# jason-li-831202/Vehicle-CV-ADAS

Hardware: NVIDIA H100
Metric: end-to-end frames/sec (YOLOv8l+UFLDv2+ByteTrack) 1280x720 (higher is better)
Workload: dtype f16

## Files before the change

vehicle-cv-adas_b200/csrc/gemm_v3.cu:

```cuda
#include "common.h"
#include <math.h>
#include <stdlib.h>
#include <string.h>
#include <mutex>
#include "tc_common.cuh"
#include "gemm_v3.h"

namespace adas {

template <bool HS>
__device__ __forceinline__ float v3_act(float x, int act) {
    if constexpr (HS) return hardswish(x);
    else return act_apply_base(x, act);
}

template <int BN, bool UP2, bool HS>
__global__ void __launch_bounds__(V3_THREADS, 1)
conv_gemm_v3_kernel(const __grid_constant__ CUtensorMap tmA, const __grid_constant__ CUtensorMap tmB, const GemmV3 g) {
    constexpr int MTX = V3_ACC_COLS / BN >= 4 ? 4 : V3_ACC_COLS / BN >= 1 ? V3_ACC_COLS / BN : 1;
    extern __shared__ uint8_t smem_raw[];
    __shared__ __align__(8) uint64_t full_bar[8];
    __shared__ __align__(8) uint64_t empty_bar[8];

    const GemmParams& p = g.p;
    const int warp_idx = threadIdx.x >> 5;
    const int lane = threadIdx.x & 31;
    const int stages = g.stages;
    const uint32_t smem_base = (smem_u32(smem_raw) + 1023u) & ~1023u;
    const int BMT = BM * g.MT;

    if (threadIdx.x == 0) {
        asm volatile("prefetch.tensormap [%0];" ::"l"(reinterpret_cast<uint64_t>(&tmA)) : "memory");
        asm volatile("prefetch.tensormap [%0];" ::"l"(reinterpret_cast<uint64_t>(&tmB)) : "memory");
        for (int s = 0; s < stages; ++s) {
            mbar_init(smem_u32(&full_bar[s]), 1);
            mbar_init(smem_u32(&empty_bar[s]), 4 * V3_CONSUMERS);
        }
        asm volatile("fence.mbarrier_init.release.cluster;" ::: "memory");
        asm volatile("fence.proxy.async.shared::cta;" ::: "memory");
    }
    __syncthreads();
    const int tps = g.slab ? 3 : 1;
    const uint32_t a_bytes = p.s2 ? (uint32_t)(p.s2_bw * p.s2_bh * BK * 2) : (uint32_t)g.a_sub_bytes;
    const uint32_t tx_bytes = (uint32_t)g.MT * a_bytes + (uint32_t)(tps * BN * BK * 2);
    const bool dx_inner = p.ntaps == 9;
    const int o_cnt = dx_inner ? 3 : p.ntaps;
    const int i_cnt = dx_inner && !g.slab ? 3 : 1;
    const int per_img = p.s2_tw * p.s2_th;
    auto load_b = [&](int grp, int kc, int n0, uint32_t stage, uint32_t fb) {
        const uint32_t b_dst = smem_base + stage * g.stage_bytes + g.MT * g.a_sub_bytes;
        for (int t = 0; t < tps; ++t) tma_load_2d(b_dst + t * g.b_bytes, &tmB, (grp + t) * p.Kc + kc * BK, n0, fb);
    };
    auto load_a = [&](int grp, int kc, int m_t, uint32_t stage, uint32_t fb) {
        const uint32_t a_dst = smem_base + stage * g.stage_bytes;
        const int m0 = m_t * BMT;
        if (p.s2) {
            const int dy = p.ntaps == 9 ? grp / 3 : 1, dx = p.ntaps == 9 ? grp % 3 : 1;
            for (int mt = 0; mt < g.MT; ++mt) {
                const int pi = m_t * g.MT + mt;
                const int b = pi / per_img;
                const int rem = pi - b * per_img;
                const int ty = rem / p.s2_tw, tx = rem - ty * p.s2_tw;
                tma_load_4d(a_dst + mt * g.a_sub_bytes, &tmA, kc * BK, 2 * tx * p.s2_bw + dx, 2 * ty * p.s2_bh + dy, b, fb);
            }
        } else {
            int shift = 0;
            if (p.ntaps == 9) shift = (grp / 3 - 1) * p.Wp + (grp % 3 - 1);
            else if (p.ntaps == 4) shift = (grp - 2) * p.Wp;
            for (int mt = 0; mt < g.MT; ++mt) tma_load_2d(a_dst + mt * g.a_sub_bytes, &tmA, kc * BK, m0 + shift + mt * BM, fb);
        }
    };
    int pre = 0;
    if (threadIdx.x == 0 && g.pdl && g.prefetch_w && (int)blockIdx.x < g.total_tiles) {
        const int steps_tile = o_cnt * p.kpt * i_cnt;
        pre = steps_tile < stages ? steps_tile : stages;
        const int n0 = ((int)blockIdx.x % g.n_tiles) * BN;
        for (int j = 0; j < pre; ++j) {
            const int in = j % i_cnt, kc = (j / i_cnt) % p.kpt, o = j / (i_cnt * p.kpt);
            const uint32_t fb = smem_u32(&full_bar[j]);
            mbar_expect_tx(fb, tx_bytes);
            load_b(dx_inner ? o * 3 + in : o, kc, n0, (uint32_t)j, fb);
        }
    }
    if (g.pdl) {
        asm volatile("griddepcontrol.wait;" ::: "memory");
        asm volatile("griddepcontrol.launch_dependents;" ::: "memory");
    }

    if (warp_idx < 4) {
        asm volatile("setmaxnreg.dec.sync.aligned.u32 40;" ::: "memory");
        if (threadIdx.x == 0) {
            uint32_t s = 0, ph = 0;
            int step = 0;
            for (int w = blockIdx.x; w < g.total_tiles; w += gridDim.x) {
                const int n_t = w % g.n_tiles, m_t = w / g.n_tiles;
                const int n0 = n_t * BN;
                for (int o = 0; o < o_cnt; ++o) {
                    for (int kc = 0; kc < p.kpt; ++kc) {
                        for (int in = 0; in < i_cnt; ++in) {
                            const int grp = dx_inner ? o * 3 + in : o;
                            const uint32_t fb = smem_u32(&full_bar[s]);
                            if (step < pre) {
                                load_a(grp, kc, m_t, s, fb);
                            } else {
                                mbar_wait(smem_u32(&empty_bar[s]), ph ^ 1u);
                                mbar_expect_tx(fb, tx_bytes);
                                load_a(grp, kc, m_t, s, fb);
                                load_b(grp, kc, n0, s, fb);
                            }
                            ++step;
                            if (++s == (uint32_t)stages) { s = 0; ph ^= 1u; }
                        }
                    }
                }
            }
        }
    } else {
        asm volatile("setmaxnreg.inc.sync.aligned.u32 232;" ::: "memory");
        const int cw = (warp_idx - 4) >> 2;
        const int wq = warp_idx & 3;
        const int nsteps = p.ntaps * p.kpt / tps;
        const size_t res_ld = (size_t)(p.res_ld < 0 ? -p.res_ld : p.res_ld);
        float acc[MTX][BN / 2];
#pragma unroll
        for (int mt = 0; mt < MTX; ++mt)
#pragma unroll
            for (int i = 0; i < BN / 2; ++i) acc[mt][i] = 0.f;
        uint32_t s = 0, ph = 0;
        for (int w = blockIdx.x; w < g.total_tiles; w += gridDim.x) {
            uint32_t prev = 0;
            for (int ks = 0; ks < nsteps; ++ks) {
                mbar_wait(smem_u32(&full_bar[s]), ph);
                const uint32_t a_base = smem_base + s * g.stage_bytes + (uint32_t)cw * (64u * 128u);
                const uint32_t b_base = smem_base + s * g.stage_bytes + g.MT * g.a_sub_bytes;
#pragma unroll
                for (int mt = 0; mt < MTX; ++mt)
#pragma unroll
                    for (int i = 0; i < BN / 2; ++i) reg_fence(acc[mt][i]);
                wgmma_fence();
                for (int t = 0; t < tps; ++t) {
                    const uint64_t bdesc = make_smem_desc(b_base + t * g.b_bytes);
#pragma unroll
                    for (int mt = 0; mt < MTX; ++mt) {
                        if (mt < g.MT) {
                            const uint64_t adesc = make_smem_desc(a_base + (uint32_t)(mt * g.a_sub_bytes + t * 128));
#pragma unroll
                            for (int k = 0; k < BK / 16; ++k)
                                WgmmaCols<0, BN>::run(acc[mt], adesc + 2u * k, bdesc + 2u * k, (uint32_t)((ks | t | k) != 0));
                        }
                    }
                }
                wgmma_commit();
                wgmma_wait<1>();
                if (ks > 0 && lane == 0) mbar_arrive(smem_u32(&empty_bar[prev]));
                prev = s;
                if (++s == (uint32_t)stages) { s = 0; ph ^= 1u; }
            }
            wgmma_wait<0>();
#pragma unroll
            for (int mt = 0; mt < MTX; ++mt)
#pragma unroll
                for (int i = 0; i < BN / 2; ++i) reg_fence(acc[mt][i]);
            if (lane == 0) mbar_arrive(smem_u32(&empty_bar[prev]));

            const int n_t = w % g.n_tiles, m_t = w / g.n_tiles;
            const int n0 = n_t * BN;
            const int m0 = m_t * BMT;
            const int c0 = 2 * (lane & 3);
            const float neg_slope = p.act == 3 ? 0.1f : 0.f;
#pragma unroll
            for (int mt = 0; mt < MTX; ++mt) {
                if (mt >= g.MT) break;
#pragma unroll
                for (int h = 0; h < 2; ++h) {
                    const int r = cw * 64 + wq * 16 + (lane >> 2) + 8 * h;
                    int row = m0 + mt * BM + r;
                    bool ok = row < p.M;
                    if (p.s2) {
                        const int pi = m_t * g.MT + mt;
                        const int b = fast_div(pi, g.fd_per_img);
                        const int rem = pi - b * per_img;
                        const int ty = fast_div(rem, g.fd_tw), tx = rem - ty * p.s2_tw;
                        const int j = fast_div(r, g.fd_bw), i = r - j * p.s2_bw;
                        const int yo = ty * p.s2_bh + j, xo = tx * p.s2_bw + i;
                        ok = (pi < g.n_patches) && (r < p.s2_bw * p.s2_bh) && (yo < p.s2_Ho) && (xo < p.s2_Wo);
                        row = (b * (p.s2_Ho + 2) + yo + 1) * (p.s2_Wo + 2) + xo + 1;
                    } else if (p.mask_H > 0 && ok) {
                        const int Wp = p.mask_W + 2;
                        const int pp = row - fast_div(row, g.fd_img) * g.fd_img.d;
                        const int yy = fast_div(pp, g.fd_wp);
                        const int xx = pp - yy * Wp;
                        ok = (yy >= 1) && (yy <= p.mask_H) && (xx >= 1) && (xx <= p.mask_W);
                    }
                    if (!ok) continue;
                    if (p.transposed) {
                        const float row_bias = p.bias != nullptr ? __ldg(p.bias + row) : 0.f;
#pragma unroll
                        for (int j = 0; j < BN / 8; ++j) {
#pragma unroll
                            for (int e = 0; e < 2; ++e) {
                                const int col = n0 + 8 * j + c0 + e;
                                if (col < p.N) {
                                    const float x = v3_act<HS>(acc[mt][4 * j + 2 * h + e] + row_bias, p.act);
                                    if (p.out_f32) reinterpret_cast<float*>(p.out)[(size_t)col * (size_t)p.out_ld + row] = x;
                                    else reinterpret_cast<__half*>(p.out)[(size_t)col * (size_t)p.out_ld + row] = __float2half_rn(x);
                                }
                            }
                        }
                        continue;
                    }
                    if constexpr (UP2) {
                        const int bi = fast_div(row, g.fd_img);
                        const int pp = row - bi * g.fd_img.d;
                        const int yy = fast_div(pp, g.fd_wp), xx = pp - yy * (p.mask_W + 2);
                        const int Wo2 = 2 * p.mask_W + 2, co = p.N >> 2;
                        const int up_row = (bi * (2 * p.mask_H + 2) + 2 * yy - 1) * Wo2 + 2 * xx - 1;
#pragma unroll
                        for (int j = 0; j < BN / 8; ++j) {
                            const int n = n0 + 8 * j + c0;
                            if (n0 + 8 * j >= p.N) break;
                            float x0 = acc[mt][4 * j + 2 * h], x1 = acc[mt][4 * j + 2 * h + 1];
                            if (p.bias != nullptr) { x0 += __ldg(p.bias + n); x1 += __ldg(p.bias + n + 1); }
                            x0 = v3_act<HS>(x0, p.act); x1 = v3_act<HS>(x1, p.act);
                            const int q = (n >= co) + (n >= 2 * co) + (n >= 3 * co);
                            const size_t o = (size_t)(up_row + (q >> 1) * Wo2 + (q & 1)) * (size_t)p.out_ld + (n - q * co);
                            if (p.out_f32) *reinterpret_cast<float2*>(reinterpret_cast<float*>(p.out) + o) = make_float2(x0, x1);
                            else *reinterpret_cast<__half2*>(reinterpret_cast<__half*>(p.out) + o) = __floats2half2_rn(x0, x1);
                        }
                        continue;
                    }
                    const __half* rp = p.res != nullptr ? p.res + (size_t)row * res_ld : nullptr;
#pragma unroll
                    for (int j = 0; j < BN / 8; ++j) {
                        const int n = n0 + 8 * j + c0;
                        if (n0 + 8 * j >= p.N) break;
                        float x0 = acc[mt][4 * j + 2 * h], x1 = acc[mt][4 * j + 2 * h + 1];
                        if (p.bias != nullptr) { x0 += __ldg(p.bias + n); x1 += __ldg(p.bias + n + 1); }
                        float2 rv = make_float2(0.f, 0.f);
                        if (rp != nullptr) rv = __half22float2(*reinterpret_cast<const __half2*>(rp + n));
                        if (p.res_ld < 0) { x0 += rv.x; x1 += rv.y; }
                        if constexpr (HS) { x0 = hardswish(x0); x1 = hardswish(x1); }
                        else if (p.act == 1) silu2(x0, x1);
                        else if (p.act >= 2) { x0 = relu_leaky(x0, neg_slope); x1 = relu_leaky(x1, neg_slope); }
                        if (p.res_ld > 0) { x0 += p.res_scale * rv.x; x1 += p.res_scale * rv.y; }
                        if (p.out_f32) *reinterpret_cast<float2*>(reinterpret_cast<float*>(p.out) + (size_t)row * (size_t)p.out_ld + n) = make_float2(x0, x1);
                        else *reinterpret_cast<__half2*>(reinterpret_cast<__half*>(p.out) + (size_t)row * (size_t)p.out_ld + n) = __floats2half2_rn(x0, x1);
                    }
                }
            }
        }
    }
}

#define V3_FOR_EACH_BN(X) X(16) X(32) X(48) X(64) X(80) X(96) X(112) X(128) X(144) X(160) X(176) X(192) X(208) X(224) X(240) X(256)

template <bool HS>
static const void* v3_kernel_act(int BN, bool up2) {
    if (up2) {
        switch (BN) {
            case 64: return reinterpret_cast<const void*>(&conv_gemm_v3_kernel<64, true, HS>);
            case 128: return reinterpret_cast<const void*>(&conv_gemm_v3_kernel<128, true, HS>);
            case 256: return reinterpret_cast<const void*>(&conv_gemm_v3_kernel<256, true, HS>);
            default: return nullptr;
        }
    }
    switch (BN) {
#define V3_CASE(b) case b: return reinterpret_cast<const void*>(&conv_gemm_v3_kernel<b, false, HS>);
        V3_FOR_EACH_BN(V3_CASE)
#undef V3_CASE
        default: return nullptr;
    }
}
static const void* v3_kernel(int BN, bool up2 = false, bool hswish = false) {
    return hswish ? v3_kernel_act<true>(BN, up2) : v3_kernel_act<false>(BN, up2);
}
static bool v3_up2_tile(int BN) { return BN == 64 || BN == 128 || BN == 256; }

struct V3Device { bool attr_set = false; int num_sms = 0; };
static std::mutex g_v3_mu;
static V3Device g_v3_dev[64];

static int v3_device_state(int* num_sms) {
    int dev = 0;
    ADAS_CUDA(cudaGetDevice(&dev));
    ADAS_CHECK(dev >= 0 && dev < 64, "device index %d out of range", dev);
    std::lock_guard<std::mutex> lk(g_v3_mu);
    V3Device& d = g_v3_dev[dev];
    if (!d.attr_set) {
        for (int hs = 0; hs < 2; ++hs) {
            for (int bn = 16; bn <= 256; bn += 16) ADAS_CUDA(cudaFuncSetAttribute(v3_kernel(bn, false, hs), cudaFuncAttributeMaxDynamicSharedMemorySize, V3_DYN_SMEM_MAX));
            for (int bn = 64; bn <= 256; bn *= 2) ADAS_CUDA(cudaFuncSetAttribute(v3_kernel(bn, true, hs), cudaFuncAttributeMaxDynamicSharedMemorySize, V3_DYN_SMEM_MAX));
        }
        ADAS_CUDA(cudaDeviceGetAttribute(&d.num_sms, cudaDevAttrMultiProcessorCount, dev));
        d.attr_set = true;
    }
    *num_sms = d.num_sms;
    return 0;
}

static FastDiv make_fastdiv(int d) {
    FastDiv f;
    f.d = d < 1 ? 1 : d;
    f.mul = 0; f.shr = 0;
    if (f.d > 1) {
        int lg = 0;
        while ((1u << lg) < (uint32_t)f.d) ++lg;
        const int p = 31 + lg;
        f.mul = (uint32_t)((((uint64_t)1 << p) + (uint64_t)f.d - 1) / (uint64_t)f.d);
        f.shr = (uint32_t)(p - 32);
    }
    return f;
}

int v3_num_sms(int* num_sms) { return v3_device_state(num_sms); }

static int env_int(const char* name, int dflt) {
    const char* v = getenv(name);
    return v ? atoi(v) : dflt;
}

int gemm_v3_config(const GemmParams& p_in, GemmV3* g) {
    GemmParams p = p_in;
    static const int force_bn = env_int("ADAS_B200_BN", 0), force_mt = env_int("ADAS_B200_MT", 0);
    if (force_bn >= 16 && force_bn <= 256 && force_bn % 16 == 0 && force_bn <= ((p.N + 15) / 16) * 16 && !p.transposed && !p.up2) p.BN = force_bn;
    if (p.BN % 16 != 0 || p.BN < 16 || p.BN > 256) return 1;
    if (p.up2 && !v3_up2_tile(p.BN)) return 1;
    g->p = p;
    g->MT = p.mt_hint >= 1 ? p.mt_hint : ((p.BN <= 128) ? 2 : 1);
    if (force_mt >= 1 && force_mt <= 4) g->MT = force_mt;
    if (g->MT > 4) return 1;
    const int mt_max = V3_ACC_COLS / p.BN < 4 ? V3_ACC_COLS / p.BN : 4;
    if (g->MT > mt_max) g->MT = mt_max;
    const int b_bytes = ((p.BN * BK * 2) + 1023) & ~1023;
    g->b_bytes = b_bytes;
    static const int no_slab_env = env_int("ADAS_B200_NOSLAB", 0);
    const int slab_stage = g->MT * SLAB_BYTES + 3 * b_bytes;
    g->slab = p.ntaps == 9 && !p.s2 && !p.no_slab && !no_slab_env && 2 * slab_stage <= V3_DYN_SMEM_MAX - 1024;
    g->a_sub_bytes = g->slab ? SLAB_BYTES : A_STAGE_BYTES;
    g->stage_bytes = g->slab ? slab_stage : g->MT * g->a_sub_bytes + b_bytes;
    int stages = (V3_DYN_SMEM_MAX - 1024) / g->stage_bytes;
    if (stages > 8) stages = 8;
    if (stages < 2) return 1;
    g->stages = stages;
    g->p.stages = stages;
    const int BMT = BM * g->MT;
    g->n_tiles = (p.N + p.BN - 1) / p.BN;
    g->m_tiles = (p.M + BMT - 1) / BMT;
    g->total_tiles = g->n_tiles * g->m_tiles;
    g->n_patches = p.s2 ? p.M / BM : 0;
    g->fd_img = make_fastdiv((p.mask_H + 2) * (p.mask_W + 2));
    g->fd_wp = make_fastdiv(p.mask_W + 2);
    g->fd_per_img = make_fastdiv(p.s2 ? p.s2_tw * p.s2_th : 1);
    g->fd_tw = make_fastdiv(p.s2 ? p.s2_tw : 1);
    g->fd_bw = make_fastdiv(p.s2 ? p.s2_bw : 1);
    g->pdl = 0;
    static const int no_prefetch = env_int("ADAS_B200_NO_WPREFETCH", 0);
    g->prefetch_w = (no_prefetch || p.transposed) ? 0 : 1;
    return 0;
}

static int v3_smem_bytes(const GemmV3& g) { return g.stages * g.stage_bytes + 1024; }

int gemm_v3_launch(const GemmV3Launch& L, cudaStream_t st) {
    int num_sms = 0;
    if (v3_device_state(&num_sms)) return 1;
    static const int pdl = env_int("ADAS_B200_PDL", 1);
    GemmV3 gp = L.g;
    gp.pdl = pdl ? 1 : 0;
    const void* fn = v3_kernel(gp.p.BN, gp.p.up2 != 0, gp.p.act == 5);
    ADAS_CHECK(fn != nullptr, "gemm_v3: no kernel for BN %d%s", gp.p.BN, gp.p.up2 ? " with the transposed-conv store" : "");
    cudaLaunchConfig_t cfg = {};
    cfg.gridDim = dim3(gp.total_tiles < num_sms ? gp.total_tiles : num_sms, 1, 1);
    cfg.blockDim = dim3(V3_THREADS, 1, 1);
    cfg.dynamicSmemBytes = v3_smem_bytes(gp);
    cfg.stream = st;
    cudaLaunchAttribute attr1;
    attr1.id = cudaLaunchAttributeProgrammaticStreamSerialization;
    attr1.val.programmaticStreamSerializationAllowed = 1;
    cfg.attrs = &attr1;
    cfg.numAttrs = pdl ? 1 : 0;
    CUtensorMap tmA = L.tmA, tmB = L.tmB;
    void* args[] = {&tmA, &tmB, &gp};
    ADAS_CUDA(cudaLaunchKernelExC(&cfg, fn, args));
    count_launch();
    return 0;
}

int gemm_v3_candidates(const GemmParams& base, int max_out, int* BN_out, int* mt_out, int* no_slab_out) {
    int num_sms = 132;
    if (v3_num_sms(&num_sms)) return 0;
    const int cand[] = {256, 192, 128, 64, 160, 96, 80, 48, 32, 16};
    struct C { double t; int BN, mt, slab; } list[64];
    int n = 0;
    const int N = base.N, ntaps = base.ntaps;
    const int kpt = (base.Kc + 63) / 64;
    for (int ci = 0; ci < 10; ++ci) {
        int BN = cand[ci];
        if (BN > N) { if (BN - N >= 64 || (BN % 64 == 0 && BN - N >= 16 && N > 64)) continue; BN = (N + 15) / 16 * 16; }
        if (BN > 256) continue;
        if (BN < 64 && N >= 64) continue;
        if (base.up2 && !v3_up2_tile(BN)) continue;
        const int n_tiles = (N + BN - 1) / BN;
        if ((double)n_tiles * BN > 1.35 * N) continue;
        bool dup = false;
        for (int k = 0; k < n; ++k) dup = dup || (list[k].BN == BN);
        if (dup) continue;
        for (int mt = 1; mt <= 4; ++mt) {
            GemmParams p = base;
            p.BN = BN; p.mt_hint = mt;
            GemmV3 g;
            if (gemm_v3_config(p, &g)) continue;
            if (g.p.BN != BN || g.MT != mt) continue;
            const double tiles = (double)g.total_tiles;
            const int tps = g.slab ? 3 : 1;
            const double bytes = (double)ntaps * kpt / tps * (g.MT * (double)g.a_sub_bytes + tps * BN * 128.0);
            const double rate = BN >= 64 ? 1.0 : 0.7;
            const double mma = (double)g.MT * ntaps * kpt * 4.0 * BN / rate;
            const double epi = (double)g.MT * 128.0 * BN * 0.12;
            const double per_tile = fmax(bytes / 32.0, mma) + epi + 400.0;
            const double waves = ceil(tiles / (double)num_sms);
            const double t = waves * per_tile + 3500.0;
            if (n < 64) { list[n].t = t; list[n].BN = BN; list[n].mt = mt; list[n].slab = g.slab; ++n; }
        }
    }
    for (int i = 1; i < n; ++i) { C c = list[i]; int j = i - 1; while (j >= 0 && list[j].t > c.t) { list[j + 1] = list[j]; --j; } list[j + 1] = c; }
    if (n == 0) { list[0].BN = N <= 256 ? (N + 15) / 16 * 16 : 256; list[0].mt = 1; list[0].slab = 0; n = 1; }
    if (base.up2 && !v3_up2_tile(list[0].BN)) list[0].BN = N >= 256 ? 256 : N >= 128 ? 128 : 64;
    int out = 0;
    for (int i = 0; i < n && out < max_out; ++i) {
        for (int ns = 0; ns <= list[i].slab && out < max_out; ++ns) {
            BN_out[out] = list[i].BN; mt_out[out] = list[i].mt; no_slab_out[out] = ns; ++out;
        }
    }
    return out;
}

int gemm_v3_prepare(const GemmParams& p, const void* a_base, uint64_t a_inner, uint64_t a_rows, uint64_t a_stride_bytes,
                    const void* b_base, uint64_t b_inner, uint64_t b_rows, uint64_t b_stride_bytes, void** opaque) {
    ADAS_CHECK(p.BN % 16 == 0 && p.BN >= 16 && p.BN <= 256, "gemm_v3: bad BN %d", p.BN);
    ADAS_CHECK(p.N % 8 == 0 || p.transposed, "gemm_v3: N %d must be a multiple of 8", p.N);
    ADAS_CHECK(!p.s2, "gemm_v3_prepare: stride-2 ops go through gemm_v3_prepare_s2");
    GemmV3Launch* L = new GemmV3Launch();
    if (gemm_v3_config(p, &L->g)) { delete L; ADAS_CHECK(false, "gemm_v3: tile does not fit (BN %d, mt %d)", p.BN, p.mt_hint); }
    if (make_tmap_2d(&L->tmA, a_base, a_inner, a_rows, a_stride_bytes, 64, L->g.slab ? SLAB_ROWS : BM) ||
        make_tmap_2d(&L->tmB, b_base, b_inner, b_rows, b_stride_bytes, 64, (uint32_t)L->g.p.BN)) {
        delete L;
        return 1;
    }
    *opaque = L;
    return 0;
}

int gemm_v3_prepare_s2(const GemmParams& p, const void* a_base, uint64_t a_C, uint64_t a_Wp, uint64_t a_Hp, uint64_t a_B, uint64_t a_ld,
                       const void* b_base, uint64_t b_inner, uint64_t b_rows, uint64_t b_stride_bytes, void** opaque) {
    ADAS_CHECK(p.s2 && p.BN % 16 == 0 && p.BN >= 16 && p.BN <= 256 && p.N % 8 == 0, "gemm_v3_s2: bad tile (BN %d)", p.BN);
    GemmV3Launch* L = new GemmV3Launch();
    if (gemm_v3_config(p, &L->g)) { delete L; ADAS_CHECK(false, "gemm_v3_s2: tile does not fit (BN %d, mt %d)", p.BN, p.mt_hint); }
    if (make_tmap_4d_s2(&L->tmA, a_base, a_C, a_Wp, a_Hp, a_B, a_ld, 2u * (uint32_t)p.s2_bw, 2u * (uint32_t)p.s2_bh) ||
        make_tmap_2d(&L->tmB, b_base, b_inner, b_rows, b_stride_bytes, 64, (uint32_t)L->g.p.BN)) {
        delete L;
        return 1;
    }
    *opaque = L;
    return 0;
}

int gemm_v3_run(void* opaque, cudaStream_t st) { return gemm_v3_launch(*static_cast<GemmV3Launch*>(opaque), st); }
void gemm_v3_free(void* opaque) { delete static_cast<GemmV3Launch*>(opaque); }
void gemm_v3_describe(const void* opaque, char* out, int cap) {
    const GemmV3& g = static_cast<const GemmV3Launch*>(opaque)->g;
    snprintf(out, (size_t)cap, "M=%d N=%d K=%d taps=%d act=%d res=%d f32=%d s2=%d tr=%d up2=%d | v3 BN=%d MT=%d slab=%d stages=%d tiles=%d wpre=%d", g.p.M,
             g.p.N, g.p.Kc * g.p.ntaps, g.p.ntaps, g.p.act, g.p.res ? (g.p.res_ld < 0 ? -1 : 1) : 0, g.p.out_f32, g.p.s2, g.p.transposed, g.p.up2,
             g.p.BN, g.MT, g.slab, g.stages, g.total_tiles, g.prefetch_w);
}

}
```

Before: 1000.0.

## Specialize consumer mainloop on compile-time MT and taps-per-stage, batch epilogue loads

Moves the WGMMA consumer path into templates specialised on the M-tile count and taps per stage (1 or 3 for slab mode), chosen by a compile-time recursive dispatch. This gives constant descriptor offsets and stage sizes, removes the runtime mt<g.MT guards, fully unrolls the tap loop and sizes the accumulator array exactly. The per-step reg_fence over all accumulators is dropped, and the epilogue now loads residual and bias values in batches of up to 8 (bias as float2) before applying them. In exchange it produces more kernel instantiations and larger binaries, and it disables slab mode for the upsample path.

```diff
diff --git a/vehicle-cv-adas_b200/csrc/gemm_v3.cu b/vehicle-cv-adas_b200/csrc/gemm_v3.cu
--- a/vehicle-cv-adas_b200/csrc/gemm_v3.cu
+++ b/vehicle-cv-adas_b200/csrc/gemm_v3.cu
@@ -14,10 +14,182 @@
     else return act_apply_base(x, act);
 }
 
+__host__ __device__ constexpr int v3_b_bytes(int BN) { return ((BN * BK * 2) + 1023) & ~1023; }
+__host__ __device__ constexpr int v3_mt_max(int BN) { return V3_ACC_COLS / BN < 4 ? V3_ACC_COLS / BN : 4; }
+__host__ __device__ constexpr int v3_slab_stage_bytes(int BN, int MT) { return MT * SLAB_BYTES + 3 * v3_b_bytes(BN); }
+__host__ __device__ constexpr bool v3_slab_fits(int BN, int MT) { return 2 * v3_slab_stage_bytes(BN, MT) <= V3_DYN_SMEM_MAX - 1024; }
+
+template <int BN, int MT, int TPS>
+__device__ __forceinline__ void v3_mainloop(float (&acc)[MT][BN / 2], uint32_t smem_base, uint32_t a_row_off, int nsteps, int stages,
+                                            uint32_t& s, uint32_t& ph, uint64_t* full_bar, uint64_t* empty_bar, int lane) {
+    constexpr uint32_t A_SUB = TPS == 3 ? SLAB_BYTES : A_STAGE_BYTES;
+    constexpr uint32_t B_BYTES = v3_b_bytes(BN);
+    constexpr uint32_t STAGE = MT * A_SUB + TPS * B_BYTES;
+    uint32_t prev = 0;
+    for (int ks = 0; ks < nsteps; ++ks) {
+        mbar_wait(smem_u32(&full_bar[s]), ph);
+        const uint32_t st = smem_base + s * STAGE;
+        const uint64_t adesc = make_smem_desc(st + a_row_off);
+        const uint64_t bdesc = make_smem_desc(st + MT * A_SUB);
+        const uint32_t scale = ks != 0;
+        wgmma_fence();
+#pragma unroll
+        for (int t = 0; t < TPS; ++t)
+#pragma unroll
+            for (int mt = 0; mt < MT; ++mt)
+#pragma unroll
+                for (int k = 0; k < BK / 16; ++k)
+                    WgmmaCols<0, BN>::run(acc[mt], adesc + (mt * A_SUB + t * 128) / 16 + 2 * k, bdesc + t * B_BYTES / 16 + 2 * k,
+                                          (t | k) != 0 ? 1u : scale);
+        wgmma_commit();
+        wgmma_wait<1>();
+        if (ks > 0 && lane == 0) mbar_arrive(smem_u32(&empty_bar[prev]));
+        prev = s;
+        if (++s == (uint32_t)stages) { s = 0; ph ^= 1u; }
+    }
+    wgmma_wait<0>();
+#pragma unroll
+    for (int mt = 0; mt < MT; ++mt)
+#pragma unroll
+        for (int i = 0; i < BN / 2; ++i) reg_fence(acc[mt][i]);
+    if (lane == 0) mbar_arrive(smem_u32(&empty_bar[prev]));
+}
+
+template <int BN, bool UP2, bool HS, int MT, int TPS>
+__device__ __forceinline__ void v3_tiles(const GemmV3& g, uint32_t smem_base, uint64_t* full_bar, uint64_t* empty_bar, int warp_idx, int lane) {
+    const GemmParams& p = g.p;
+    const int cw = (warp_idx - 4) >> 2;
+    const int wq = warp_idx & 3;
+    const int nsteps = p.ntaps * p.kpt / TPS;
+    const int per_img = p.s2_tw * p.s2_th;
+    const size_t res_ld = (size_t)(p.res_ld < 0 ? -p.res_ld : p.res_ld);
+    float acc[MT][BN / 2];
+#pragma unroll
+    for (int mt = 0; mt < MT; ++mt)
+#pragma unroll
+        for (int i = 0; i < BN / 2; ++i) acc[mt][i] = 0.f;
+    uint32_t s = 0, ph = 0;
+    for (int w = blockIdx.x; w < g.total_tiles; w += gridDim.x) {
+        v3_mainloop<BN, MT, TPS>(acc, smem_base, (uint32_t)cw * (64u * 128u), nsteps, g.stages, s, ph, full_bar, empty_bar, lane);
+
+        const int n_t = w % g.n_tiles, m_t = w / g.n_tiles;
+        const int n0 = n_t * BN;
+        const int m0 = m_t * (BM * MT);
+        const int c0 = 2 * (lane & 3);
+        const float neg_slope = p.act == 3 ? 0.1f : 0.f;
+#pragma unroll
+        for (int mt = 0; mt < MT; ++mt) {
+#pragma unroll
+            for (int h = 0; h < 2; ++h) {
+                const int r = cw * 64 + wq * 16 + (lane >> 2) + 8 * h;
+                int row = m0 + mt * BM + r;
+                bool ok = row < p.M;
+                if (p.s2) {
+                    const int pi = m_t * MT + mt;
+                    const int b = fast_div(pi, g.fd_per_img);
+                    const int rem = pi - b * per_img;
+                    const int ty = fast_div(rem, g.fd_tw), tx = rem - ty * p.s2_tw;
+                    const int j = fast_div(r, g.fd_bw), i = r - j * p.s2_bw;
+                    const int yo = ty * p.s2_bh + j, xo = tx * p.s2_bw + i;
+                    ok = (pi < g.n_patches) && (r < p.s2_bw * p.s2_bh) && (yo < p.s2_Ho) && (xo < p.s2_Wo);
+                    row = (b * (p.s2_Ho + 2) + yo + 1) * (p.s2_Wo + 2) + xo + 1;
+                } else if (p.mask_H > 0 && ok) {
+                    const int Wp = p.mask_W + 2;
+                    const int pp = row - fast_div(row, g.fd_img) * g.fd_img.d;
+                    const int yy = fast_div(pp, g.fd_wp);
+                    const int xx = pp - yy * Wp;
+                    ok = (yy >= 1) && (yy <= p.mask_H) && (xx >= 1) && (xx <= p.mask_W);
+                }
+                if (!ok) continue;
+                if (p.transposed) {
+                    const float row_bias = p.bias != nullptr ? __ldg(p.bias + row) : 0.f;
+#pragma unroll
+                    for (int j = 0; j < BN / 8; ++j) {
+#pragma unroll
+                        for (int e = 0; e < 2; ++e) {
+                            const int col = n0 + 8 * j + c0 + e;
+                            if (col < p.N) {
+                                const float x = v3_act<HS>(acc[mt][4 * j + 2 * h + e] + row_bias, p.act);
+                                if (p.out_f32) reinterpret_cast<float*>(p.out)[(size_t)col * (size_t)p.out_ld + row] = x;
+                                else reinterpret_cast<__half*>(p.out)[(size_t)col * (size_t)p.out_ld + row] = __float2half_rn(x);
+                            }
+                        }
+                    }
+                    continue;
+                }
+                if constexpr (UP2) {
+                    const int bi = fast_div(row, g.fd_img);
+                    const int pp = row - bi * g.fd_img.d;
+                    const int yy = fast_div(pp, g.fd_wp), xx = pp - yy * (p.mask_W + 2);
+                    const int Wo2 = 2 * p.mask_W + 2, co = p.N >> 2;
+                    const int up_row = (bi * (2 * p.mask_H + 2) + 2 * yy - 1) * Wo2 + 2 * xx - 1;
+#pragma unroll
+                    for (int j = 0; j < BN / 8; ++j) {
+                        const int n = n0 + 8 * j + c0;
+                        if (n0 + 8 * j >= p.N) break;
+                        float x0 = acc[mt][4 * j + 2 * h], x1 = acc[mt][4 * j + 2 * h + 1];
+                        if (p.bias != nullptr) { x0 += __ldg(p.bias + n); x1 += __ldg(p.bias + n + 1); }
+                        x0 = v3_act<HS>(x0, p.act); x1 = v3_act<HS>(x1, p.act);
+                        const int q = (n >= co) + (n >= 2 * co) + (n >= 3 * co);
+                        const size_t o = (size_t)(up_row + (q >> 1) * Wo2 + (q & 1)) * (size_t)p.out_ld + (n - q * co);
+                        if (p.out_f32) *reinterpret_cast<float2*>(reinterpret_cast<float*>(p.out) + o) = make_float2(x0, x1);
+                        else *reinterpret_cast<__half2*>(reinterpret_cast<__half*>(p.out) + o) = __floats2half2_rn(x0, x1);
+                    }
+                    continue;
+                }
+                const __half* rp = p.res != nullptr ? p.res + (size_t)row * res_ld : nullptr;
+                constexpr int RB = BN / 8 < 8 ? BN / 8 : 8;
+#pragma unroll
+                for (int j0 = 0; j0 < BN / 8; j0 += RB) {
+                    if (n0 + 8 * j0 >= p.N) break;
+                    __half2 rq[RB];
+                    float2 bq[RB];
+#pragma unroll
+                    for (int jj = 0; jj < RB; ++jj) {
+                        const int j = j0 + jj;
+                        const bool in = j < BN / 8 && n0 + 8 * j < p.N;
+                        rq[jj] = __float2half2_rn(0.f);
+                        bq[jj] = make_float2(0.f, 0.f);
+                        if (rp != nullptr && in) rq[jj] = *reinterpret_cast<const __half2*>(rp + n0 + 8 * j + c0);
+                        if (p.bias != nullptr && in) bq[jj] = __ldg(reinterpret_cast<const float2*>(p.bias + n0 + 8 * j + c0));
+                    }
+#pragma unroll
+                    for (int jj = 0; jj < RB; ++jj) {
+                        const int j = j0 + jj;
+                        if (j >= BN / 8) break;
+                        const int n = n0 + 8 * j + c0;
+                        if (n0 + 8 * j >= p.N) break;
+                        float x0 = acc[mt][4 * j + 2 * h], x1 = acc[mt][4 * j + 2 * h + 1];
+                        if (p.bias != nullptr) { x0 += bq[jj].x; x1 += bq[jj].y; }
+                        const float2 rv = __half22float2(rq[jj]);
+                        if (p.res_ld < 0) { x0 += rv.x; x1 += rv.y; }
+                        if constexpr (HS) { x0 = hardswish(x0); x1 = hardswish(x1); }
+                        else if (p.act == 1) silu2(x0, x1);
+                        else if (p.act >= 2) { x0 = relu_leaky(x0, neg_slope); x1 = relu_leaky(x1, neg_slope); }
+                        if (p.res_ld > 0) { x0 += p.res_scale * rv.x; x1 += p.res_scale * rv.y; }
+                        if (p.out_f32) *reinterpret_cast<float2*>(reinterpret_cast<float*>(p.out) + (size_t)row * (size_t)p.out_ld + n) = make_float2(x0, x1);
+                        else *reinterpret_cast<__half2*>(reinterpret_cast<__half*>(p.out) + (size_t)row * (size_t)p.out_ld + n) = __floats2half2_rn(x0, x1);
+                    }
+                }
+            }
+        }
+    }
+}
+
+template <int BN, bool UP2, bool HS, int MT>
+__device__ __forceinline__ void v3_consumers(const GemmV3& g, uint32_t smem_base, uint64_t* full_bar, uint64_t* empty_bar, int warp_idx, int lane) {
+    if constexpr (MT < v3_mt_max(BN)) {
+        if (g.MT != MT) { v3_consumers<BN, UP2, HS, MT + 1>(g, smem_base, full_bar, empty_bar, warp_idx, lane); return; }
+    }
+    if constexpr (!UP2 && v3_slab_fits(BN, MT)) {
+        if (g.slab) { v3_tiles<BN, UP2, HS, MT, 3>(g, smem_base, full_bar, empty_bar, warp_idx, lane); return; }
+    }
+    v3_tiles<BN, UP2, HS, MT, 1>(g, smem_base, full_bar, empty_bar, warp_idx, lane);
+}
+
 template <int BN, bool UP2, bool HS>
 __global__ void __launch_bounds__(V3_THREADS, 1)
 conv_gemm_v3_kernel(const __grid_constant__ CUtensorMap tmA, const __grid_constant__ CUtensorMap tmB, const GemmV3 g) {
-    constexpr int MTX = V3_ACC_COLS / BN >= 4 ? 4 : V3_ACC_COLS / BN >= 1 ? V3_ACC_COLS / BN : 1;
     extern __shared__ uint8_t smem_raw[];
     __shared__ __align__(8) uint64_t full_bar[8];
     __shared__ __align__(8) uint64_t empty_bar[8];
@@ -117,138 +289,7 @@
         }
     } else {
         asm volatile("setmaxnreg.inc.sync.aligned.u32 232;" ::: "memory");
-        const int cw = (warp_idx - 4) >> 2;
-        const int wq = warp_idx & 3;
-        const int nsteps = p.ntaps * p.kpt / tps;
-        const size_t res_ld = (size_t)(p.res_ld < 0 ? -p.res_ld : p.res_ld);
-        float acc[MTX][BN / 2];
-#pragma unroll
-        for (int mt = 0; mt < MTX; ++mt)
-#pragma unroll
-            for (int i = 0; i < BN / 2; ++i) acc[mt][i] = 0.f;
-        uint32_t s = 0, ph = 0;
-        for (int w = blockIdx.x; w < g.total_tiles; w += gridDim.x) {
-            uint32_t prev = 0;
-            for (int ks = 0; ks < nsteps; ++ks) {
-                mbar_wait(smem_u32(&full_bar[s]), ph);
-                const uint32_t a_base = smem_base + s * g.stage_bytes + (uint32_t)cw * (64u * 128u);
-                const uint32_t b_base = smem_base + s * g.stage_bytes + g.MT * g.a_sub_bytes;
-#pragma unroll
-                for (int mt = 0; mt < MTX; ++mt)
-#pragma unroll
-                    for (int i = 0; i < BN / 2; ++i) reg_fence(acc[mt][i]);
-                wgmma_fence();
-                for (int t = 0; t < tps; ++t) {
-                    const uint64_t bdesc = make_smem_desc(b_base + t * g.b_bytes);
-#pragma unroll
-                    for (int mt = 0; mt < MTX; ++mt) {
-                        if (mt < g.MT) {
-                            const uint64_t adesc = make_smem_desc(a_base + (uint32_t)(mt * g.a_sub_bytes + t * 128));
-#pragma unroll
-                            for (int k = 0; k < BK / 16; ++k)
-                                WgmmaCols<0, BN>::run(acc[mt], adesc + 2u * k, bdesc + 2u * k, (uint32_t)((ks | t | k) != 0));
-                        }
-                    }
-                }
-                wgmma_commit();
-                wgmma_wait<1>();
-                if (ks > 0 && lane == 0) mbar_arrive(smem_u32(&empty_bar[prev]));
-                prev = s;
-                if (++s == (uint32_t)stages) { s = 0; ph ^= 1u; }
-            }
-            wgmma_wait<0>();
-#pragma unroll
-            for (int mt = 0; mt < MTX; ++mt)
-#pragma unroll
-                for (int i = 0; i < BN / 2; ++i) reg_fence(acc[mt][i]);
-            if (lane == 0) mbar_arrive(smem_u32(&empty_bar[prev]));
-
-            const int n_t = w % g.n_tiles, m_t = w / g.n_tiles;
-            const int n0 = n_t * BN;
-            const int m0 = m_t * BMT;
-            const int c0 = 2 * (lane & 3);
-            const float neg_slope = p.act == 3 ? 0.1f : 0.f;
-#pragma unroll
-            for (int mt = 0; mt < MTX; ++mt) {
-                if (mt >= g.MT) break;
-#pragma unroll
-                for (int h = 0; h < 2; ++h) {
-                    const int r = cw * 64 + wq * 16 + (lane >> 2) + 8 * h;
-                    int row = m0 + mt * BM + r;
-                    bool ok = row < p.M;
-                    if (p.s2) {
-                        const int pi = m_t * g.MT + mt;
-                        const int b = fast_div(pi, g.fd_per_img);
-                        const int rem = pi - b * per_img;
-                        const int ty = fast_div(rem, g.fd_tw), tx = rem - ty * p.s2_tw;
-                        const int j = fast_div(r, g.fd_bw), i = r - j * p.s2_bw;
-                        const int yo = ty * p.s2_bh + j, xo = tx * p.s2_bw + i;
-                        ok = (pi < g.n_patches) && (r < p.s2_bw * p.s2_bh) && (yo < p.s2_Ho) && (xo < p.s2_Wo);
-                        row = (b * (p.s2_Ho + 2) + yo + 1) * (p.s2_Wo + 2) + xo + 1;
-                    } else if (p.mask_H > 0 && ok) {
-                        const int Wp = p.mask_W + 2;
-                        const int pp = row - fast_div(row, g.fd_img) * g.fd_img.d;
-                        const int yy = fast_div(pp, g.fd_wp);
-                        const int xx = pp - yy * Wp;
-                        ok = (yy >= 1) && (yy <= p.mask_H) && (xx >= 1) && (xx <= p.mask_W);
-                    }
-                    if (!ok) continue;
-                    if (p.transposed) {
-                        const float row_bias = p.bias != nullptr ? __ldg(p.bias + row) : 0.f;
-#pragma unroll
-                        for (int j = 0; j < BN / 8; ++j) {
-#pragma unroll
-                            for (int e = 0; e < 2; ++e) {
-                                const int col = n0 + 8 * j + c0 + e;
-                                if (col < p.N) {
-                                    const float x = v3_act<HS>(acc[mt][4 * j + 2 * h + e] + row_bias, p.act);
-                                    if (p.out_f32) reinterpret_cast<float*>(p.out)[(size_t)col * (size_t)p.out_ld + row] = x;
-                                    else reinterpret_cast<__half*>(p.out)[(size_t)col * (size_t)p.out_ld + row] = __float2half_rn(x);
-                                }
-                            }
-                        }
-                        continue;
-                    }
-                    if constexpr (UP2) {
-                        const int bi = fast_div(row, g.fd_img);
-                        const int pp = row - bi * g.fd_img.d;
-                        const int yy = fast_div(pp, g.fd_wp), xx = pp - yy * (p.mask_W + 2);
-                        const int Wo2 = 2 * p.mask_W + 2, co = p.N >> 2;
-                        const int up_row = (bi * (2 * p.mask_H + 2) + 2 * yy - 1) * Wo2 + 2 * xx - 1;
-#pragma unroll
-                        for (int j = 0; j < BN / 8; ++j) {
-                            const int n = n0 + 8 * j + c0;
-                            if (n0 + 8 * j >= p.N) break;
-                            float x0 = acc[mt][4 * j + 2 * h], x1 = acc[mt][4 * j + 2 * h + 1];
-                            if (p.bias != nullptr) { x0 += __ldg(p.bias + n); x1 += __ldg(p.bias + n + 1); }
-                            x0 = v3_act<HS>(x0, p.act); x1 = v3_act<HS>(x1, p.act);
-                            const int q = (n >= co) + (n >= 2 * co) + (n >= 3 * co);
-                            const size_t o = (size_t)(up_row + (q >> 1) * Wo2 + (q & 1)) * (size_t)p.out_ld + (n - q * co);
-                            if (p.out_f32) *reinterpret_cast<float2*>(reinterpret_cast<float*>(p.out) + o) = make_float2(x0, x1);
-                            else *reinterpret_cast<__half2*>(reinterpret_cast<__half*>(p.out) + o) = __floats2half2_rn(x0, x1);
-                        }
-                        continue;
-                    }
-                    const __half* rp = p.res != nullptr ? p.res + (size_t)row * res_ld : nullptr;
-#pragma unroll
-                    for (int j = 0; j < BN / 8; ++j) {
-                        const int n = n0 + 8 * j + c0;
-                        if (n0 + 8 * j >= p.N) break;
-                        float x0 = acc[mt][4 * j + 2 * h], x1 = acc[mt][4 * j + 2 * h + 1];
-                        if (p.bias != nullptr) { x0 += __ldg(p.bias + n); x1 += __ldg(p.bias + n + 1); }
-                        float2 rv = make_float2(0.f, 0.f);
-                        if (rp != nullptr) rv = __half22float2(*reinterpret_cast<const __half2*>(rp + n));
-                        if (p.res_ld < 0) { x0 += rv.x; x1 += rv.y; }
-                        if constexpr (HS) { x0 = hardswish(x0); x1 = hardswish(x1); }
-                        else if (p.act == 1) silu2(x0, x1);
-                        else if (p.act >= 2) { x0 = relu_leaky(x0, neg_slope); x1 = relu_leaky(x1, neg_slope); }
-                        if (p.res_ld > 0) { x0 += p.res_scale * rv.x; x1 += p.res_scale * rv.y; }
-                        if (p.out_f32) *reinterpret_cast<float2*>(reinterpret_cast<float*>(p.out) + (size_t)row * (size_t)p.out_ld + n) = make_float2(x0, x1);
-                        else *reinterpret_cast<__half2*>(reinterpret_cast<__half*>(p.out) + (size_t)row * (size_t)p.out_ld + n) = __floats2half2_rn(x0, x1);
-                    }
-                }
-            }
-        }
+        v3_consumers<BN, UP2, HS, 1>(g, smem_base, full_bar, empty_bar, warp_idx, lane);
     }
 }
 
@@ -329,13 +370,12 @@
     g->MT = p.mt_hint >= 1 ? p.mt_hint : ((p.BN <= 128) ? 2 : 1);
     if (force_mt >= 1 && force_mt <= 4) g->MT = force_mt;
     if (g->MT > 4) return 1;
-    const int mt_max = V3_ACC_COLS / p.BN < 4 ? V3_ACC_COLS / p.BN : 4;
-    if (g->MT > mt_max) g->MT = mt_max;
-    const int b_bytes = ((p.BN * BK * 2) + 1023) & ~1023;
+    if (g->MT > v3_mt_max(p.BN)) g->MT = v3_mt_max(p.BN);
+    const int b_bytes = v3_b_bytes(p.BN);
     g->b_bytes = b_bytes;
     static const int no_slab_env = env_int("ADAS_B200_NOSLAB", 0);
-    const int slab_stage = g->MT * SLAB_BYTES + 3 * b_bytes;
-    g->slab = p.ntaps == 9 && !p.s2 && !p.no_slab && !no_slab_env && 2 * slab_stage <= V3_DYN_SMEM_MAX - 1024;
+    const int slab_stage = v3_slab_stage_bytes(p.BN, g->MT);
+    g->slab = p.ntaps == 9 && !p.s2 && !p.up2 && !p.no_slab && !no_slab_env && v3_slab_fits(p.BN, g->MT);
     g->a_sub_bytes = g->slab ? SLAB_BYTES : A_STAGE_BYTES;
     g->stage_bytes = g->slab ? slab_stage : g->MT * g->a_sub_bytes + b_bytes;
     int stages = (V3_DYN_SMEM_MAX - 1024) / g->stage_bytes;
```

After: 1242 (median of 6 runs). +24.2%, better.
